# MaxRamgraber/Triangular-Transport-Toolbox

Measured on AMD Instinct MI355X. Metric: map-evals/sec (forward+inverse, N samples x D comps), higher is better.
Workload: dtype f64; 1 GPU; C5: d=40 banded separable map, order 3, N=1e6 (Gaussian-mixture target); N_per_gpu=1000000, D=40, columns=40, inverse=table, layout=column-major resident in HBM, coefficients=reference-optimised (tests/golden), world_size=1

## Files before the change

### triangular_transport_toolbox_amd/csrc/ttm_band.h

```cpp
#pragma once

#include <stdint.h>

#include "../../include/ttm.h"

namespace ttm_band {

int build_records(const ttm_program* p, double* U, void* stream);

int record_stride(int cls, int lag);

bool usable(const ttm_program* p, int k0, int k1);

int forward(const ttm_program* p, const double* U, int k0, int k1, const double* Xsoa, int64_t ldx, int64_t N, double* Zsoa,
            int64_t ldz, double* logdet, const double* sigma, double* sumsq, int cus, size_t lds_per_cu, int block, int resident, void* stream,
            const char** kernel_name);

int inverse(const ttm_program* p, const double* U, int k0, int k1, const double* Zsoa, int64_t ldz, double* Xsoa, int64_t ldx,
            int64_t N, const double* tab_x, int T, const double* y_affine, const double* tmin, const double* tmax, const int32_t* bkt,
            int nb, const double* img, int img_doubles, int cus, size_t lds_per_cu, int window, int block, int resident, void* stream,
            const char** kernel_name);

int newton(const ttm_program* p, const double* U, int k0, int k1, const double* Zsoa, int64_t ldz, double* Xsoa, int64_t ldx, int64_t N,
           int32_t* iters, int cus, size_t lds_per_cu, int block, void* stream, const char** kernel_name);

int bisect(const ttm_program* p, const double* U, int k0, int k1, const double* Zsoa, int64_t ldz, double* Xsoa, int64_t ldx, int64_t N,
           int32_t* iters, int cus, size_t lds_per_cu, int block, void* stream, const char** kernel_name);

bool bisect_plans(const ttm_program* p, const double* U, int k0, int k1, const double* Zsoa, int64_t ldz, double* Xsoa, int64_t ldx, int64_t N,
                  int32_t* iters, int cus, size_t lds_per_cu, int block);

int score(const ttm_program* p, const double* U, const double* Xsoa, int64_t ldx, int64_t N, double* Gsoa, int64_t ldg, const double* g_scale,
          const double* ld_affine, int cus, size_t lds_per_cu, int block, void* stream, const char** kernel_name);

int roundtrip(const ttm_program* p, const double* U, int k0, int k1, const double* Xsoa, int64_t ldx, int64_t N, double* Zsoa, int64_t ldz,
              double* Xr, int64_t ldr, double* logdet, const double* sigma, double* sumsq, const double* tab_x, int T, const double* y_affine,
// ... 9 lines not shown
```

### triangular_transport_toolbox_amd/csrc/ttm_band.hip

```cpp
#include <hip/hip_runtime.h>
#include <math.h>
#include <stdint.h>
#include <stdlib.h>
#include <type_traits>
#include <utility>

#include "ttm_band.h"
#include "ttm_band_etab.h"
#include "ttm_band_image.h"
#include "ttm_band_policy.h"

namespace ttm_band {

typedef const __attribute__((address_space(4))) double* cdbl_p;
typedef const __attribute__((address_space(4))) int* cint_p;
struct __attribute__((aligned(16))) D2 { double x, y; };

__device__ const double g_band_etab[2 * TTM_BAND_ET_N] = { TTM_BAND_ETAB_VALUES };
__device__ double g_band_taylor[6] = {1.0 / 5040.0, 1.0 / 720.0, 1.0 / 120.0, 1.0 / 24.0, 1.0 / 6.0, 0.5};

__host__ __device__ constexpr int cls_db(int cls) { return cls == 1 ? 3 : (cls == 2 ? 5 : (cls == 3 ? 7 : 10)); }
__host__ __device__ constexpr int cls_da(int cls) { return cls == 1 ? 1 : (cls == 2 ? 5 : (cls == 3 ? 7 : 10)); }
__host__ __device__ constexpr int cls_gs(int cls) { return cls == 1 ? 8 : (cls == 2 ? 16 : 24); }
__host__ __device__ constexpr int cls_gp(int cls) { return cls_db(cls) + 1 + cls_da(cls); }
__host__ __device__ constexpr int rec_stride(int cls, int lag) { return (TTM_P_HDR + lag * cls_gp(cls) + 7) / 8 * 8; }

#define BAND_ET_DOUBLES (2 * TTM_BAND_ET_N)
#define BAND_CT 1024
#define BAND_NS 4
#define BAND_PF 1
static_assert(BAND_POLICY_TILE_ROWS == BAND_NS * BAND_CT && BAND_POLICY_HALF_ROWS == 2 * BAND_CT && BAND_NS == 4,
              "ttm_band_policy.h counts the rows of pair slot 0 of these tiles");

__device__ __forceinline__ void band_dma16(const void* g, unsigned int lds_wave_base) {
    asm volatile("s_mov_b32 m0, %1\n\ts_nop 0\n\tglobal_load_lds_dwordx4 %0, off" ::"v"(g), "s"(lds_wave_base) : "m0");
}
__device__ __forceinline__ unsigned int band_lds_addr(const void* p) {
    return (unsigned int)(uintptr_t)(const __attribute__((address_space(3))) void*)p;
}

template <bool WAIT = true>
__device__ __forceinline__ void band_stage(double* lds_dst, const double* src, int n) {
    const int units = n >> 1;
    const unsigned int base = band_lds_addr(lds_dst);
    for (int u0 = 0; u0 < units; u0 += BAND_CT) {
        const int u = u0 + (int)threadIdx.x;
        if (u < units) band_dma16(src + 2 * (size_t)u, __builtin_amdgcn_readfirstlane(base + (unsigned int)(u0 + ((int)threadIdx.x & ~63)) * 16u));
    }
    if (WAIT) asm volatile("s_waitcnt vmcnt(0)" ::: "memory");
}
// ... 964 lines not shown
};

__device__ __forceinline__ void band_ring_fill(const double* img, int ncomp, double* tabs, int tab_slot, int n) {
    const int U = tab_slot >> 1;
    const int total = n * U;
    for (int u0 = 0; u0 < total; u0 += BAND_CT) {
        const int u = u0 + (int)threadIdx.x;
        if (u < total) {
            const int t = u / U, o = u - t * U;
            band_dma16(img + (size_t)(t % ncomp) * tab_slot + 2 * o,
                       __builtin_amdgcn_readfirstlane(band_lds_addr(tabs) + (unsigned int)(u0 + ((int)threadIdx.x & ~63)) * 16u));
        }
    }
}

template <int CLS, int LAG, bool RING = false, int G = 0, int POL = 0>
__device__ __forceinline__ void band_inverse_tile(const BandInvCtx& cx, bool full, int kb, int ke, const char* zcol, char* xcol, unsigned int tbase,
                                                  const unsigned int (&roff)[BAND_NS / 2], double (&pend)[BAND_NS][LAG],
                                                  const D2 (&zfirst)[BAND_NS / 2], bool have_first, BandRing* rg = nullptr) {
    constexpr int DB = cls_db(CLS), DA = cls_da(CLS), PS = rec_stride(CLS, LAG);
    constexpr int NS = BAND_NS, NP = NS / 2, HALF = 2 * BAND_CT;
    cdbl_p rec = cx.P + (int64_t)(kb + LAG) * PS;
    cdbl_p kt = cx.kt;
    const double* slot = RING ? cx.tabs + (size_t)rg->pos * cx.tab_slot : cx.tabs;
    const double ystep = cx.ystep;
    const int nb1 = cx.nb - 1;
    D2 za[NP], zb[NP];
    if (have_first) {
#pragma unroll
        for (int q = 0; q < NP; ++q) za[q] = zfirst[q];
    } else {
        band_slots<NP>([&](auto Q) { constexpr int q = decltype(Q)::value; za[q] = band_load2<band_z_nt<POL, q>>(zcol + roff[q]); });
    }
    auto interp = [&](double y_lo, double y_hi, double x_lo, double x_hi, double e_lo, double tgt, double& rr, double& ee) {
        const double dx = fmax(x_hi - x_lo, 1e-300);
        double rc = __builtin_amdgcn_rcp(dx);
        rc = fma(fma(-dx, rc, 1.0), rc, rc);
        const double delta = ((y_hi - y_lo) * rc) * (tgt - x_lo);
        rr = delta + y_lo;
        const double w = (delta * -0.25) * (y_lo + rr);
        double p = fma(kt[0], w, kt[1]);
        p = fma(p, w, kt[2]);
        p = fma(p, w, kt[3]);
        p = fma(p, w, kt[4]);
        p = fma(p, w, kt[5]);
        p = fma(p, w, 1.0);
        p = fma(p, w, 1.0);
        ee = e_lo * p;
    };
    auto step = [&](int j, const D2 (&zc)[NP], D2 (&zn)[NP]) {
        {
            const char* znext = j + 1 < ke ? zcol + cx.ldzb : zcol;
            band_slots<NP>([&](auto Q) { constexpr int q = decltype(Q)::value; zn[q] = band_load2<band_z_nt<POL, q>>(znext + roff[q]); });
        }
        double start = rec[1];
        double gc[LAG * (DB + 1 + DA)];
#pragma unroll
        for (int i = 0; i < LAG * (DB + 1 + DA); ++i) gc[i] = rec[TTM_P_HDR + i];
        asm volatile("" : "+s"(start));
#pragma unroll
        for (int i = 0; i < LAG * (DB + 1 + DA); ++i) asm volatile("" : "+s"(gc[i]));
        __builtin_amdgcn_sched_barrier(0);
        double wl, wh, scale, bias;
        { const D2 a = *(const D2*)slot; wl = a.x; wh = a.y; const D2 b = *(const D2*)(slot + 2); scale = b.x; bias = b.y; }
        const lds_p xsl = band_lds(slot + BAND_RT_HDR) - 8 * cx.w0;
        const lds_p bkl = band_lds(slot + BAND_RT_HDR + cx.Weven);
        const bool deg = __builtin_amdgcn_readfirstlane(((const int*)slot)[10]) != 0;
        const int per = __builtin_amdgcn_readfirstlane(((const int*)slot)[8]);
        double traw[NS], tg[NS], r[NS], E[NS];
        unsigned long long outl = deg ? ~0ull : 0ull;
#pragma unroll
        for (int e = 0; e < NS; ++e) {
            const double z = (e & 1) ? zc[e >> 1].y : zc[e >> 1].x;
            traw[e] = z - pend[e][0];
            tg[e] = fmin(fmax(traw[e], wl), wh);
            outl |= __builtin_amdgcn_ballot_w64(traw[e] != tg[e]);
        }
        if (RING && G > 0) {
            band_dma16(rg->src + (size_t)rg->tcomp * rg->stride, rg->tabs_lds + (unsigned int)rg->tpos * rg->stride + rg->dst);
            if (++rg->tpos == rg->R) rg->tpos = 0;
            if (++rg->tcomp == rg->ncomp) rg->tcomp = 0;
        }
        auto search = [&](auto nc) {
            constexpr int NC = decltype(nc)::value;
            int pos[NS];
#pragma unroll
            for (int e = 0; e < NS; ++e) {
                const int bi = min((int)fma(tg[e], scale, bias), nb1);
                pos[e] = (int)*(const __attribute__((address_space(3))) unsigned short*)(bkl + 2 * bi);
            }
            double qv[NS][NC];
#pragma unroll
            for (int e = 0; e < NS; ++e) {
                const lds_p q4 = xsl + 8 * pos[e];
                qv[e][0] = band_lds_f64(q4);
#pragma unroll
// ... 41 lines not shown
#pragma unroll
            for (int q = 0; q < NP; ++q) {
                band_store2<POL != 0>(xcol + (size_t)((tbase + (unsigned int)(q * HALF)) * 8u), r[2 * q], r[2 * q + 1]);
            }
        } else {
#pragma unroll
            for (int q = 0; q < NP; ++q) {
                const unsigned int n = tbase + (unsigned int)(q * HALF);
                const D2 o = {r[2 * q], r[2 * q + 1]};
                char* xp = xcol + (size_t)(n * 8u);
                if (n + 1 < cx.c1_32) { if (POL != 0) band_store2<true>(xp, o.x, o.y); else *(D2*)xp = o; }
                else if (n < cx.c1_32) *(double*)xp = o.x;
            }
        }
        rec += PS; slot += cx.tab_slot; zcol += cx.ldzb; xcol += cx.ldxb;
        if (RING) {
            if (++rg->pos == rg->R) { rg->pos = 0; slot = cx.tabs; }
            if (G > 0 && ++rg->gcnt == G) {
                rg->gcnt = 0;
                static_assert(G == 0 || G == 4, "the counted wait below is 3 G - 2");
                asm volatile("s_waitcnt vmcnt(10)" ::: "memory");
                __syncthreads();
            }
        }
    };
    int j = kb;
    for (; j + 1 < ke; j += 2) {
        step(j, za, zb);
        step(j + 1, zb, za);
    }
    if (j < ke) step(j, za, zb);
}

template <int CLS, int LAG, int KM>
__global__ __launch_bounds__(BAND_CT) void k_band_inverse(const double* __restrict__ U_, int64_t p_off, int k0, int k1, int kcol0,
                                                          const double* __restrict__ Z, int64_t ldz, double* X, int64_t ldx, int64_t N,
                                                          const double* __restrict__ tab_x, int T, double y0, double ystep, double ylast,
                                                          const double* __restrict__ tmin, const double* __restrict__ tmax,
                                                          const int* __restrict__ bkt, int nb, int tab_slot, int B, int64_t rows_per_wg,
                                                          int w0, int W) {
    constexpr int DB = cls_db(CLS), DA = cls_da(CLS), PS = rec_stride(CLS, LAG);
    constexpr int NS = BAND_NS, NP = NS / 2, CT = BAND_CT, ROWS = NS * CT, HALF = 2 * CT;
    extern __shared__ __align__(16) double g_lds[];
    const int tid = threadIdx.x;
    const int64_t c0 = (int64_t)blockIdx.x * rows_per_wg;
    if (c0 >= N) return;
// ... 129 lines not shown
                    for (int q = 0; q < NP; ++q) {
                        D2 xv = {0.0, 0.0};
                        if (cc >= 0) xv = *(const D2*)(col + roff[q]);
                        band_push<DB, DA, LAG>(rec + TTM_P_HDR, rec[1], xv.x, cc >= 0 ? band_expq_series(xv.x) : 1.0, pend[2 * q]);
                        band_push<DB, DA, LAG>(rec + TTM_P_HDR, rec[1], xv.y, cc >= 0 ? band_expq_series(xv.y) : 1.0, pend[2 * q + 1]);
                    }
                }
            }
            const char* zcol = (const char*)Z + (int64_t)(kb - k0) * ldzb;
            char* xcol = (char*)X + (int64_t)colb * ldxb;
            band_inverse_tile<CLS, LAG>(cx, full, kb, ke, zcol, xcol, tbase, roff, pend, zfirst, tile == 0);
        }
    }
}

template <int CLS, int LAG, int G, int POL = 0>
__global__ __launch_bounds__(BAND_CT) void k_band_inverse_ring(const double* __restrict__ U_, int64_t p_off, int k0, int k1, int kcol0,
                                                               const double* __restrict__ Z, int64_t ldz, double* X, int64_t ldx, int64_t N,
                                                               const double* __restrict__ tab_x, int T, double y0, double ystep, double ylast,
                                                               const double* __restrict__ tmin, const double* __restrict__ tmax,
                                                               const double* __restrict__ img, int nb, int tab_slot, int R,
                                                               int64_t rows_per_wg, int w0, int W) {
    constexpr int DB = cls_db(CLS), DA = cls_da(CLS), PS = rec_stride(CLS, LAG);
    constexpr int NS = BAND_NS, NP = NS / 2, CT = BAND_CT, ROWS = NS * CT, HALF = 2 * CT;
    extern __shared__ __align__(16) double g_lds[];
    const int tid = threadIdx.x;
    const int64_t c0 = (int64_t)blockIdx.x * rows_per_wg;
    if (c0 >= N) return;
    const int64_t c1 = c0 + rows_per_wg < N ? c0 + rows_per_wg : N;
    const int ntile = (int)((c1 - c0 + ROWS - 1) / ROWS);
    const int ncomp = k1 - k0;
// ... 10 lines not shown
    cx.T = T; cx.nb = nb; cx.tab_slot = tab_slot; cx.w0 = w0; cx.Weven = Weven; cx.k0 = k0;
    cx.y0 = y0; cx.ystep = ystep; cx.ylast = ylast; cx.ldzb = ldzb; cx.ldxb = ldxb; cx.c1_32 = (unsigned int)c1;
    BandRing rg;
    {
        const int U = tab_slot >> 1, nw = (U + 63) >> 6;
        const int piece = (tid >> 6) % nw;
        const int start = 64 * piece < U - 64 ? 64 * piece : U - 64;
        rg.src = (const char*)img + (size_t)(start + (tid & 63)) * 16;
        rg.dst = __builtin_amdgcn_readfirstlane((unsigned int)start * 16u);
        rg.tabs_lds = band_lds_addr(tabs);
        rg.stride = (unsigned int)tab_slot * 8u;
        rg.R = R; rg.ncomp = ncomp; rg.pos = 0; rg.gcnt = 0;
        rg.tpos = G > 0 ? R - G : 0;
        rg.tcomp = G > 0 ? (R - G) % ncomp : 0;
    }
    D2 zfirst[NP];
    band_slots<NP>([&](auto Q) {
        constexpr int q = decltype(Q)::value;
        unsigned int n = (unsigned int)c0 + 2u * (unsigned int)tid + (unsigned int)(q * HALF);
        n = n < last_pair ? n : last_pair;
        zfirst[q] = band_load2<band_z_nt<POL, q>>((const char*)Z + (size_t)(n * 8u));
    });
    band_ring_fill(img, ncomp, tabs, tab_slot, R);
    for (int i = tid; i < W; i += CT) {
        etab[2 * i] = band_expq_series(w0 + i == T - 1 ? ylast : (double)(w0 + i) * ystep + y0);
        etab[2 * i + 1] = w0 + i == T - 1 ? ylast : (double)(w0 + i) * ystep + y0;
    }
    asm volatile("s_waitcnt vmcnt(0)" ::: "memory");
    __syncthreads();
    for (int tile = 0; tile < ntile; ++tile) {
        const unsigned int tbase = (unsigned int)c0 + (unsigned int)tile * (unsigned int)ROWS + 2u * (unsigned int)tid;
        const bool full = c0 + (int64_t)(tile + 1) * ROWS <= c1;
        unsigned int roff[NP];
#pragma unroll
        for (int q = 0; q < NP; ++q) {
            unsigned int n = tbase + (unsigned int)(q * HALF);
            n = n < last_pair ? n : last_pair;
            roff[q] = n * 8u;
        }
        double pend[NS][LAG];
#pragma unroll
        for (int e = 0; e < NS; ++e)
#pragma unroll
            for (int l = 0; l < LAG; ++l) pend[e][l] = 0.0;
        for (int i = 0; i < LAG; ++i) {
            const int cc = kcol0 - LAG + i;
            cdbl_p rec = P + (int64_t)(k0 + i) * PS;
            const char* col = (const char*)X + (int64_t)(cc < 0 ? 0 : cc) * ldxb;
#pragma unroll
            for (int q = 0; q < NP; ++q) {
                D2 xv = {0.0, 0.0};
                if (cc >= 0) xv = *(const D2*)(col + roff[q]);
                band_push<DB, DA, LAG>(rec + TTM_P_HDR, rec[1], xv.x, cc >= 0 ? band_expq_series(xv.x) : 1.0, pend[2 * q]);
                band_push<DB, DA, LAG>(rec + TTM_P_HDR, rec[1], xv.y, cc >= 0 ? band_expq_series(xv.y) : 1.0, pend[2 * q + 1]);
            }
        }
        band_inverse_tile<CLS, LAG, true, G, POL>(cx, full, k0, k1, (const char*)Z, (char*)X + (int64_t)kcol0 * ldxb, tbase, roff, pend, zfirst, tile == 0, &rg);
    }
}

template <int CLS, int LAG, int LAGE, bool PLAIN>
__global__ __launch_bounds__(BAND_CT) void k_band_few_inverse(const double* __restrict__ U_, int64_t p_off, int k0, int k1, int kcol0,
                                                              const double* __restrict__ Z, int64_t ldz, double* X, int64_t ldx, int64_t N,
                                                              const double* __restrict__ tab_x, int T, double y0, double ystep, double ylast,
                                                              const double* __restrict__ tmin, const double* __restrict__ tmax,
                                                              const int* __restrict__ bkt, int nb, int tab_slot, int ntiles) {
    constexpr int DB = cls_db(CLS), DA = cls_da(CLS), GP = cls_gp(CLS), PS = rec_stride(CLS, LAG);
    constexpr int NS = BAND_FEW_NS, NP = NS / 2, CT = BAND_CT, ROWS = NS * CT, HALF = 2 * CT, FD = TTM_P_FEW_D, HDR = BAND_RT_HDR;
    extern __shared__ __align__(16) double g_lds[];
    const int tid = threadIdx.x;
    const int nc = k1 - k0;
// ... 1213 lines not shown
template <class F> static auto with_reach(int lag, int lage, F f) {
    if (lag == 5) return f(int_c<5>{}, int_c<5>{});
    if (lag == 3) return lage == 1 ? f(int_c<3>{}, int_c<1>{}) : lage == 2 ? f(int_c<3>{}, int_c<2>{}) : f(int_c<3>{}, int_c<3>{});
    return lage == 1 ? f(int_c<2>{}, int_c<1>{}) : f(int_c<2>{}, int_c<2>{});
}

static bool vec_ok(const void* ptr) { return (uintptr_t)ptr % 16 == 0; }
static bool col_ok(const void* ptr, int64_t ld, int64_t need) { return vec_ok(ptr) && ld % 2 == 0 && ld >= need; }
static int64_t even_rows(int64_t N) { return (N + 1) & ~(int64_t)1; }
static bool y_affine_ok(const double* y) {
    if (!y) return false;
    const double ymax = fabs(y[0]) > fabs(y[2]) ? fabs(y[0]) : fabs(y[2]);
    return y[1] > 0.0 && y[1] * ymax * 0.5 <= 0.1;
}

static int64_t chunk_rows(int64_t N, int cus) {
    const int64_t rows = (N + cus - 1) / cus;
    return (rows + 31) / 32 * 32;
}
struct ChunkGrid { int64_t rows, grid; };
static ChunkGrid chunk_grid(int64_t N, int cus) {
    const int64_t rows = chunk_rows(N, cus);
    return {rows, (N + rows - 1) / rows};
}

int record_stride(int cls, int lag) { return rec_stride(cls, lag); }

bool usable(const ttm_program* p, int k0, int k1) {
    return p && p->u_enabled && (p->u_p_lag == 2 || ((p->u_p_lag == 3 || p->u_p_lag == TTM_P_LAG_MAX) && p->D <= TTM_P_FEW_D)) && p->u_h_cls >= 1 &&
           (p->u_h_cls <= 3 || (p->u_h_cls == 4 && p->D <= TTM_P_FEW_D)) &&
           p->h_ucomp && k0 >= 0 && k1 <= p->D && k0 < k1 && p->u_p_stride == rec_stride(p->u_h_cls, p->u_p_lag);
}

static int uc(const ttm_program* p, int k, int word) { return p->h_ucomp[k * TTM_UC_LEN + word]; }
// ... 69 lines not shown
static size_t block_lds_span(const ttm_program* p, int k0, int k1, int Bc, bool splines_only) {
    size_t lds = 0;
    for (int kb = k0; kb < k1; kb += Bc) {
        int a = kb, b = (kb + Bc < k1 ? kb + Bc : k1) - 1;
        if (splines_only) {
            while (a <= b && uc(p, a, TTM_UC_NI) <= 0) ++a;
            while (b >= a && uc(p, b, TTM_UC_NI) <= 0) --b;
        }
        const size_t s = a > b ? 0 : (size_t)(uc(p, b, TTM_UC_TAB_OFF) + TTM_U_TSTRIDE * uc(p, b, TTM_UC_NI) - uc(p, a, TTM_UC_TAB_OFF)) * 8;
        lds = s > lds ? s : lds;
    }
    return lds;
}

int forward(const ttm_program* p, const double* U, int k0, int k1, const double* Xsoa, int64_t ldx, int64_t N, double* Zsoa, int64_t ldz,
            double* logdet, const double* sigma, double* sumsq, int cus, size_t lds_per_cu, int block, int resident, void* stream,
            const char** kernel_name) {
    if (!usable(p, k0, k1) || (!Zsoa && !logdet && !sumsq) || N >= ((int64_t)1 << 28)) return 1;
    if (!col_ok(Xsoa, ldx, even_rows(N)) || (Zsoa && !col_ok(Zsoa, ldz, 0)) || !vec_ok(U) || !vec_ok(logdet) || !vec_ok(sumsq)) return 1;
    const bool dens = logdet || sumsq;
    const size_t stat = dens ? (size_t)BAND_UNI * 8 : 0;
    if (dens && k1 - k0 > BAND_UNI) return 1;
    const size_t fixed = (size_t)BAND_ET_DOUBLES * 8 + stat;
    if (lds_per_cu <= fixed) return 1;
    const int Bc = plan_blocks(p, k0, k1, lds_per_cu - fixed, block);
    if (Bc <= 0) return 1;
    const size_t lds = block_lds_sum(p, k0, k1, Bc) + fixed - stat;
    const int cls = p->u_h_cls, lag = p->u_p_lag, kcol0 = uc(p, k0, TTM_UC_KC);
    if (logdet && !Zsoa && !sumsq && k1 - k0 <= BAND_UNI) {
        const size_t lbudget = lds_per_cu - (size_t)BAND_UNI * 8;
        const int LBc = plan_blocks(p, k0, k1, lbudget, block);
        const size_t llds = LBc > 0 ? block_lds_span(p, k0, k1, LBc, true) + 16 : 0;
// ... 23 lines not shown
                          ldx, N, Zsoa, ldz, logdet, sigma, sumsq, fs.ntiles, fs.tab0, fs.ntab);
        }
    }
    if (lag != 2 || cls > 3) return 1;
    const bool own = sweep_has_own(p, k0, k1);
    const ChunkGrid cg = chunk_grid(N, cus);
    if (dens) {
        auto dk = with_bool(Zsoa != nullptr, [&](auto WZ) {
            return with_bool(own, [&](auto OW) {
                return with_cls<3>(cls, [&](auto C) { return k_band_density<decltype(C)::value, 2, decltype(WZ)::value, decltype(OW)::value>; });
            });
        });
        return launch(dk, cg.grid, lds, stream, "k_band_density", kernel_name, U, p->u_p_off, k0, k1, kcol0, Xsoa, ldx, N, Zsoa, ldz, logdet, sigma,
                      sumsq, cg.rows, Bc);
    }
    const bool pol = (band_resident_policy(N, cg.rows, k1 - k0, resident) & BAND_POLICY_FORWARD) != 0;
    auto kern = with_bool(pol, [&](auto PO) {
        return with_bool(own, [&](auto OW) {
            return with_cls<3>(cls, [&](auto C) { return k_band_forward<decltype(C)::value, 2, decltype(OW)::value, decltype(PO)::value ? 1 : 0>; });
        });
    });
    return launch(kern, cg.grid, lds, stream, "k_band_forward", kernel_name, U, p->u_p_off, k0, k1, kcol0, Xsoa, ldx, N, Zsoa, ldz, cg.rows, Bc);
}

int roundtrip(const ttm_program* p, const double* U, int k0, int k1, const double* Xsoa, int64_t ldx, int64_t N, double* Zsoa, int64_t ldz,
              double* Xr, int64_t ldr, double* logdet, const double* sigma, double* sumsq, const double* tab_x, int T, const double* y_affine,
              const double* tmin, const double* tmax, const int32_t* bkt, int nb, int cus, size_t lds_per_cu, bool force, void* stream,
              const char** kernel_name) {
    const int nc = k1 - k0;
    if (!usable(p, k0, k1) || nc > TTM_P_FEW_D || !Xr || T < 64 || T + 4 > BAND_CT || nb + 1 != 1024 || N >= ((int64_t)1 << 28)) return 1;
    if (!vec_ok(bkt) || (sigma && !logdet) || !y_affine_ok(y_affine)) return 1;
    const int64_t need = even_rows(N);
    if (!col_ok(Xsoa, ldx, need) || (Zsoa && !col_ok(Zsoa, ldz, need)) || !col_ok(Xr, ldr, need) || !vec_ok(U) || !vec_ok(logdet) || !vec_ok(sumsq))
        return 1;
    const FewSweep fs = few_sweep(p, k0, k1, N, cus);
    const BandImageSlot slot = band_image_slot(T, nb);
    const size_t lds = slot.lds(nc) + fs.lds;
// ... 76 lines not shown
static BlockPlan block_plan(int T, int W, int nb, int ncomp, size_t lds_per_cu, int block) {
    const BandImageSlot slot = band_image_slot(W, nb);
    BlockPlan b = {W, (T - W) / 2, slot.tab_slot, 0, 0, 0};
    if (slot.lds(1) > lds_per_cu) return b;
    b.Bc = (int)((lds_per_cu - slot.lds(0)) / ((size_t)slot.tab_slot * 8));
    if (b.Bc > ncomp) b.Bc = ncomp;
    if (b.Bc > BAND_RT_KMAX) b.Bc = BAND_RT_KMAX;
    if (block > 0 && block < b.Bc) b.Bc = block;
    b.nblk = (ncomp + b.Bc - 1) / b.Bc;
    b.lds = slot.lds(b.Bc);
    return b;
}

int inverse(const ttm_program* p, const double* U, int k0, int k1, const double* Zsoa, int64_t ldz, double* Xsoa, int64_t ldx, int64_t N,
            const double* tab_x, int T, const double* y_affine, const double* tmin, const double* tmax, const int32_t* bkt, int nb, const double* img,
            int img_doubles, int cus, size_t lds_per_cu, int window, int block, int resident, void* stream, const char** kernel_name) {
    if (!usable(p, k0, k1) || T < 64 || T > 4096 || nb + 1 != 1024 || N >= ((int64_t)1 << 28)) return 1;
    if (!vec_ok(bkt) || !y_affine_ok(y_affine)) return 1;
    if (!col_ok(Zsoa, ldz, even_rows(N)) || !col_ok(Xsoa, ldx, even_rows(N))) return 1;
    const int ncomp = k1 - k0, cls = p->u_h_cls, lag = p->u_p_lag, kcol0 = uc(p, k0, TTM_UC_KC);
    if (ncomp <= TTM_P_FEW_D && T + 4 <= BAND_CT && window <= 0) {
        const BandImageSlot slot = band_image_slot(T, nb);
        const FewSweep fs = few_sweep(p, k0, k1, N, cus);
        if (slot.lds(ncomp) <= lds_per_cu && fs.lage <= lag) {
            auto fk = with_reach(lag, fs.lage, [&](auto L, auto E) {
                return with_bool(fs.plain, [&](auto PL) {
                    return with_cls<4>(cls, [&](auto C) {
                        return k_band_few_inverse<decltype(C)::value, decltype(L)::value, decltype(E)::value, decltype(PL)::value>;
                    });
                });
            });
            return launch(fk, fs.grid, slot.lds(ncomp), stream, "k_band_few_inverse", kernel_name, U, p->u_p_off, k0, k1, kcol0, Zsoa, ldz, Xsoa, ldx,
                          N, tab_x, T, y_affine[0], y_affine[1], y_affine[2], tmin, tmax, bkt, nb, slot.tab_slot, fs.ntiles);
        }
    }
    if (lag != 2 || cls > 3) return 1;
    const ChunkGrid cg = chunk_grid(N, cus);
    BandRingPlan pl;
    if (img && vec_ok(img) && band_ring_plan(T, nb, ncomp, lds_per_cu, window, block, BAND_WFRAC, &pl) &&
        pl.tab_slot == img_doubles) {
        const bool pol = (band_resident_policy(N, cg.rows, ncomp, resident) & BAND_POLICY_INVERSE) != 0;
        auto rk = with_bool(pol, [&](auto PO) {
            return with_bool(pl.G == 4, [&](auto G4) {
                return with_cls<3>(cls, [&](auto C) {
                    return k_band_inverse_ring<decltype(C)::value, 2, decltype(G4)::value ? 4 : 0, decltype(PO)::value ? 1 : 0>;
                });
            });
        });
        return launch(rk, cg.grid, pl.lds, stream, "k_band_inverse_ring", kernel_name, U, p->u_p_off, k0, k1, kcol0, Zsoa, ldz, Xsoa, ldx, N, tab_x, T,
                      y_affine[0], y_affine[1], y_affine[2], tmin, tmax, img, nb, pl.tab_slot, pl.R, cg.rows, pl.w0, pl.W);
    }
    BlockPlan b = block_plan(T, T, nb, ncomp, lds_per_cu, block);
    if (window != 0 && (window > 0 || (b.Bc > 0 && b.nblk > 1))) {
        int W = window > 0 ? (window < 16 ? 16 : window) : (int)(BAND_WFRAC * T);
        if (W >= T) W = T - 1;
        const BlockPlan w = block_plan(T, W, nb, ncomp, lds_per_cu, block);
        if (w.Bc > 0 && (window > 0 || w.nblk < b.nblk)) b = w;
    }
    if (b.Bc <= 0) return 1;
    auto kern = with_cls<3>(cls, [&](auto C) { return k_band_inverse<decltype(C)::value, 2, BAND_RT_KMAX>; });
    return launch(kern, cg.grid, b.lds, stream, "k_band_inverse", kernel_name, U, p->u_p_off, k0, k1, kcol0, Zsoa, ldz, Xsoa, ldx, N, tab_x, T,
                  y_affine[0], y_affine[1], y_affine[2], tmin, tmax, bkt, nb, b.tab_slot, b.Bc, cg.rows, b.w0, b.W);
}

int score(const ttm_program* p, const double* U, const double* Xsoa, int64_t ldx, int64_t N, double* Gsoa, int64_t ldg, const double* g_scale,
// ... 30 lines not shown
```

### triangular_transport_toolbox_amd/csrc/ttm_band_image.h

```cpp
#pragma once

#include <math.h>
#include <stddef.h>
#include <stdint.h>

#define BAND_RT_HDR 6
#define BAND_RING_KMAX 24

struct BandImageSlot {
    int Weven, tab_slot;
    size_t lds(int slots) const { return ((size_t)2 * Weven + (size_t)slots * tab_slot) * 8; }
};
static inline BandImageSlot band_image_slot(int W, int nb) {
    const int Weven = (W + 4 + 1) & ~1;
    return {Weven, BAND_RT_HDR + Weven + (((nb + 1 + 3) / 4 + 1) & ~1)};
}

struct BandRingPlan {
    int W, w0, Weven, tab_slot;
    int R, G;
    size_t lds;
};

static inline bool band_ring_plan(int T, int nb, int ncomp, size_t lds_per_cu, int window, int block, double wfrac, BandRingPlan* pl) {
// ... 19 lines not shown
    pl->W = W; pl->w0 = w0;
    const BandImageSlot slot = band_image_slot(W, nb);
    pl->Weven = slot.Weven; pl->tab_slot = slot.tab_slot;
    if (pl->tab_slot % 2) return false;
    if (ncomp <= B) { pl->R = ncomp; pl->G = 0; }
    else {
        const int G = 4;
        const int R = B / G * G;
        if (R < 3 * G) return false;
        pl->R = R; pl->G = G;
    }
    pl->lds = slot.lds(pl->R);
    return true;
}

#if defined(__HIPCC__)
__device__ __forceinline__ void band_bucket_params(double lo, double hi, int nb, double& scale, double& bias) {
    scale = (double)nb / (hi - lo);
    if (!(scale > 0.0 && scale < 1.0e300)) scale = 0.0;
    bias = -lo * scale;
}

__device__ inline void band_image_write(const double* xs, const int* bks, int* red, int T, int nb, double lo, double hi, int w0, int W,
                                        int Weven, int tab_slot, double* __restrict__ img) {
    const int tid = threadIdx.x, nt = blockDim.x;
    if (tid == 0) *red = 0;
    __syncthreads();
    int per = 0;
    for (int b = tid; b < nb; b += nt) {
        const int b0 = bks[b] & 0xffff, b1 = bks[b + 1] & 0xffff;
// ... 31 lines not shown
```

### triangular_transport_toolbox_amd/csrc/ttm_band_policy.h

```cpp
#pragma once

#include <stdint.h>

constexpr int64_t TTM_LLC_BYTES = (int64_t)256 << 20;

constexpr int BAND_POLICY_TILE_ROWS = 4096;
constexpr int BAND_POLICY_HALF_ROWS = 2048;

constexpr int BAND_POLICY_FORWARD = 1;
constexpr int BAND_POLICY_INVERSE = 2;

static inline int64_t band_policy_resident_rows(int64_t N, int64_t chunk_rows) {
    if (N <= 0 || chunk_rows <= 0) return 0;
    auto of_chunk = [](int64_t n) {
        const int64_t tail = n % BAND_POLICY_TILE_ROWS;
        return n / BAND_POLICY_TILE_ROWS * BAND_POLICY_HALF_ROWS + (tail < BAND_POLICY_HALF_ROWS ? tail : BAND_POLICY_HALF_ROWS);
    };
    const int64_t whole = N / chunk_rows;
    return whole * of_chunk(chunk_rows) + of_chunk(N - whole * chunk_rows);
}

static inline int band_resident_policy(int64_t N, int64_t chunk_rows, int ncomp, int option) {
    if (option >= 0) return option & (BAND_POLICY_FORWARD | BAND_POLICY_INVERSE);
    const int64_t col = 8 * (int64_t)ncomp;
    if (col * N <= TTM_LLC_BYTES) return 0;
    if (band_policy_resident_rows(N, chunk_rows) * col > TTM_LLC_BYTES) return 0;
    return BAND_POLICY_FORWARD | BAND_POLICY_INVERSE;
}
```

### triangular_transport_toolbox_amd/csrc/ttm_kernels.hip

```cpp

#include <hip/hip_runtime.h>
#include <mutex>

#include <stdio.h>
#include <stdlib.h>
#include <string.h>

#include <type_traits>

#include "ttm_eval.h"
#include "ttm_dev.h"
#include "ttm_dense.h"
#include "ttm_sample_logq.h"
#include "ttm_rng.h"
#include "ttm_uform.h"
#include "ttm_score.h"
#include "ttm_band.h"
#include "ttm_band_image.h"
#include "ttm_int.h"
#include "ttm_options.h"

using namespace ttm;


// ... 3192 lines not shown
        const int chunk = (k1 - k0 + nchunk - 1) / nchunk;
        if (ibd && ttm_int::forward(p, dev_prog(p), k0, k1, coef, fold, Xsoa, ldx, N, Zsoa, ldz, logdet, sigma, sumsq, tiles, chunk, ibd,
                                    lds_bytes(nsl, ibd, 0, 1), tuning().int_xprog != 0, stream, &name) == TTM_OK)
            return check_launch(name);
    }
    if (sep && u_on(p) && all_fast(p, k0, k1) && N < ((int64_t)1 << 29)) {
        int tab_cap = 0;
        for (int k = k0; k < k1; ++k) {
            const int c = TTM_U_TSTRIDE * p->h_ucomp[k * TTM_UC_LEN + TTM_UC_NI];
            tab_cap = c > tab_cap ? c : tab_cap;
        }
        const int ways = plan_ways_of(p);
        if (band_forward_gate(p, k0, k1, N)) {
            const char* name = nullptr;
            if (ttm_band::forward(p, fold + fold_base_size(p), k0, k1, Xsoa, ldx, N, Zsoa, ldz, logdet, sigma, sumsq, band_cus(),
                                  device_info().lds_per_cu, tuning().rt_block, tuning().band_resident, stream, &name) == 0)
                return check_launch(name);
        }
        {
            int nimax = 0, nchmax = 0;
            for (int k = k0; k < k1; ++k) {
                const int ni = p->h_ucomp[k * TTM_UC_LEN + TTM_UC_NI];
                nimax = ni > nimax ? ni : nimax;
            }
            nchmax = (nimax * TTM_U_TSTRIDE * 8 + 1023) >> 10;
            const int tab_slot = TTM_U_TSTRIDE * nimax;
            int xlead = 3, tlead = 2;
            const Tuning& tn = tuning();
            int hNS = 4;
            if (tn.hl_ns > 0) hNS = tn.hl_ns == 4 ? 4 : 2;
            const bool hot = hot_sweepable(p) && !tn.u_no_hot;
// ... 245 lines not shown
                      int64_t ldz, double* Xsoa, int64_t ldx, int64_t N, const double* tab_x, const double* tab_y, int64_t ldy,
                      int32_t T, const double* h_y_affine, const double* tmin, const double* tmax, const int32_t* bkt, int32_t nb,
                      int32_t truncate, const double* img, int64_t img_doubles, void* stream) {
    int rc = validate(p, k0, k1);
    if (rc) return rc;
    if (!coef || !fold || !Zsoa || !Xsoa || !tab_x || !tab_y || !tmin || !tmax || !bkt || N < 1 || ldx < N || ldz < N || T < 2 ||
        T < 8 || T > 65536 || nb < 4 || nb > 65536 || (ldy != 0 && ldy < T) || (h_y_affine && ldy != 0))
        return set_err(TTM_E_ARG, "ttm_inverse_table: bad arguments%s");
    if (p->monotonicity != TTM_MONO_SEPARABLE) return set_err(TTM_E_UNSUPPORTED, "table inverse needs separable monotonicity%s");
    const Tuning& tn = tuning();
    const bool affine = h_y_affine && ldy == 0;
    if (affine && truncate && band_inverse_gate(p, k0, k1, N, T, nb)) {
        const char* name = nullptr;
        if (ttm_band::inverse(p, fold + fold_base_size(p), k0, k1, Zsoa, ldz, Xsoa, ldx, N, tab_x, (int)T, h_y_affine, tmin, tmax, bkt, (int)nb,
                              tn.band_ring != 0 ? img : nullptr, (int)img_doubles, band_cus(), device_info().lds_per_cu, tn.rt_window, tn.rt_block,
                              tn.band_resident, stream, &name) == 0)
            return check_launch(name);
    }
    if (affine && rt_inverse_gate(p, k0, k1, N, T, nb) && hot_sweepable(p) && (k1 - k0 >= 4 || tn.u_loader == 1)) {
        const DeviceInfo& di = device_info();
        const int ways = plan_ways_of(p);
        const int ncomp = k1 - k0;
        int NS = tn.rt_ns == 4 ? 4 : 2;
        int W = T, w0 = 0;
        int Weven = (W + 4 + 1) & ~1;
        int tab_slot = TTM_RT_HDR + Weven + (((nb + 1 + 3) / 4 + 1) & ~1);
        const double ymax = fabs(h_y_affine[0]) > fabs(h_y_affine[2]) ? fabs(h_y_affine[0]) : fabs(h_y_affine[2]);
        const bool etab = truncate && h_y_affine[1] > 0.0 && h_y_affine[1] * ymax * 0.5 <= 0.1;
        const bool aligned = ((uintptr_t)Zsoa % 16 == 0) && (ldz % 2 == 0) && ldz >= ((N + 1) & ~(int64_t)1) &&
                             ((uintptr_t)Xsoa % 16 == 0) && (ldx % 2 == 0) && ldx >= ((N + 1) & ~(int64_t)1);
        bool band = p->u_h_ng == 2 && tn.rt_band != 0;
// ... 686 lines not shown
```

### triangular_transport_toolbox_amd/csrc/ttm_options.h

```cpp
#pragma once

#include <string.h>

#define TTM_OPTIONS(X)                                                                                                   \
    X(no_plan, 0)         \
    X(no_uform, 0)        \
    X(u_no_hot, 0)        \
    X(u_loader, -1)       \
    X(forward_ns, -1)     \
    X(inverse_ns, -1)     \
    X(u_ns, -1)           \
    X(hl_ns, -1)          \
    X(rt_off, 0)          \
    X(rt_ns, -1)          \
    X(rt_block, -1)       \
    X(rt_band, -1)        \
    X(rt_window, -1)      \
    X(gram_mfma, -1)      \
    X(band_fwd, -1)       \
    X(band_inv, -1)       \
    X(band_cus, -1)       \
    X(band_ring, -1)      \
    X(band_newton, -1)    \
    X(band_bisect, -1)    \
    X(band_score, -1)     \
    X(band_resident, -1)  \
    X(int_dense, -1)      \
    X(int_xprog, -1)      \
    X(fold_fused, -1)     \
    X(table_fused, -1)    \
    X(setup_fused, -1)    \
    X(select_coop, -1)    \
    X(colstats_one, -1)   \
    X(sep_sentinel, -1)   \
    X(sep_server, -1)     \
    X(wscan_reread, -1)   \
    X(roundtrip_fused, -1)

struct Tuning {
#define X(name, dflt) int name = dflt;
    TTM_OPTIONS(X)
// ... 10 lines not shown
```

Baseline: 162.6 billion map-evals/s.

## Add full-tile row cut and LDS-staged Z prefetch for band ring inverse

Adds a launch cut that gives each workgroup exactly one full tile of rows when the tile count nearly matches the CU count. This lets the forward and ring-inverse kernels take the full-tile code path instead of partial chunks. Also adds an opt-in variant of the ring inverse that double-buffers Z columns into LDS with async global-to-LDS loads and counted waits, trading ring slots for LDS space. The Z-DMA path and the ring-slot override are off by default; the full-tile cut is on by default, at the cost of slightly fewer workgroups than CUs.

```diff
diff --git a/triangular_transport_toolbox_amd/csrc/ttm_band.h b/triangular_transport_toolbox_amd/csrc/ttm_band.h
--- a/triangular_transport_toolbox_amd/csrc/ttm_band.h
+++ b/triangular_transport_toolbox_amd/csrc/ttm_band.h
@@ -13,13 +13,13 @@
 bool usable(const ttm_program* p, int k0, int k1);
 
 int forward(const ttm_program* p, const double* U, int k0, int k1, const double* Xsoa, int64_t ldx, int64_t N, double* Zsoa,
-            int64_t ldz, double* logdet, const double* sigma, double* sumsq, int cus, size_t lds_per_cu, int block, int resident, void* stream,
-            const char** kernel_name);
+            int64_t ldz, double* logdet, const double* sigma, double* sumsq, int cus, size_t lds_per_cu, int block, int resident, int full_tiles,
+            void* stream, const char** kernel_name);
 
 int inverse(const ttm_program* p, const double* U, int k0, int k1, const double* Zsoa, int64_t ldz, double* Xsoa, int64_t ldx,
             int64_t N, const double* tab_x, int T, const double* y_affine, const double* tmin, const double* tmax, const int32_t* bkt,
-            int nb, const double* img, int img_doubles, int cus, size_t lds_per_cu, int window, int block, int resident, void* stream,
-            const char** kernel_name);
+            int nb, const double* img, int img_doubles, int cus, size_t lds_per_cu, int window, int block, int resident, int full_tiles, int zdma,
+            int ring_slots, void* stream, const char** kernel_name);
 
 int newton(const ttm_program* p, const double* U, int k0, int k1, const double* Zsoa, int64_t ldz, double* Xsoa, int64_t ldx, int64_t N,
            int32_t* iters, int cus, size_t lds_per_cu, int block, void* stream, const char** kernel_name);
diff --git a/triangular_transport_toolbox_amd/csrc/ttm_band.hip b/triangular_transport_toolbox_amd/csrc/ttm_band.hip
--- a/triangular_transport_toolbox_amd/csrc/ttm_band.hip
+++ b/triangular_transport_toolbox_amd/csrc/ttm_band.hip
@@ -34,6 +34,9 @@
 
 __device__ __forceinline__ void band_dma16(const void* g, unsigned int lds_wave_base) {
     asm volatile("s_mov_b32 m0, %1\n\ts_nop 0\n\tglobal_load_lds_dwordx4 %0, off" ::"v"(g), "s"(lds_wave_base) : "m0");
+}
+__device__ __forceinline__ void band_dma16_nt(const void* g, unsigned int lds_wave_base) {
+    asm volatile("s_mov_b32 m0, %1\n\ts_nop 0\n\tglobal_load_lds_dwordx4 %0, off nt" ::"v"(g), "s"(lds_wave_base) : "m0");
 }
 __device__ __forceinline__ unsigned int band_lds_addr(const void* p) {
     return (unsigned int)(uintptr_t)(const __attribute__((address_space(3))) void*)p;
@@ -1028,10 +1031,17 @@
     }
 }
 
-template <int CLS, int LAG, bool RING = false, int G = 0, int POL = 0>
+#define BAND_ZD_BUF (BAND_NS * BAND_CT * 8)
+static_assert(2 * BAND_ZD_BUF == BAND_ZDMA_LDS_BYTES, "ttm_band_policy.h counts the LDS of these two buffers");
+template <int POL, int Q>
+__device__ __forceinline__ void band_zd_request(const char* g, unsigned int lds_wave_base) {
+    if (band_z_nt<POL, Q>) band_dma16_nt(g, lds_wave_base); else band_dma16(g, lds_wave_base);
+}
+template <int CLS, int LAG, bool RING = false, int G = 0, int POL = 0, int ZD = 0>
 __device__ __forceinline__ void band_inverse_tile(const BandInvCtx& cx, bool full, int kb, int ke, const char* zcol, char* xcol, unsigned int tbase,
                                                   const unsigned int (&roff)[BAND_NS / 2], double (&pend)[BAND_NS][LAG],
-                                                  const D2 (&zfirst)[BAND_NS / 2], bool have_first, BandRing* rg = nullptr) {
+                                                  const D2 (&zfirst)[BAND_NS / 2], bool have_first, BandRing* rg = nullptr, unsigned int zq = 0) {
+    static_assert(ZD == 0 || (RING && POL == 1), "ZD = 1: the ring kernel under the resident policy");
     constexpr int DB = cls_db(CLS), DA = cls_da(CLS), PS = rec_stride(CLS, LAG);
     constexpr int NS = BAND_NS, NP = NS / 2, HALF = 2 * BAND_CT;
     cdbl_p rec = cx.P + (int64_t)(kb + LAG) * PS;
@@ -1040,7 +1050,16 @@
     const double ystep = cx.ystep;
     const int nb1 = cx.nb - 1;
     D2 za[NP], zb[NP];
-    if (have_first) {
+    auto zrd = [&]() {
+        unsigned int a;
+        asm volatile("v_mbcnt_lo_u32_b32 %0, -1, 0\n\tv_mbcnt_hi_u32_b32 %0, -1, %0\n\tv_lshl_add_u32 %0, %0, 4, %1" : "=&v"(a) : "s"(zq));
+        return (lds_p)(uintptr_t)a;
+    };
+    if (ZD) {
+#pragma unroll
+        for (int q = 0; q < NP; ++q) za[q] = band_lds_pair(zrd() + q * 1024);
+        asm volatile("s_waitcnt lgkmcnt(0)" ::: "memory");
+    } else if (have_first) {
 #pragma unroll
         for (int q = 0; q < NP; ++q) za[q] = zfirst[q];
     } else {
@@ -1062,8 +1081,14 @@
         p = fma(p, w, 1.0);
         ee = e_lo * p;
     };
-    auto step = [&](int j, const D2 (&zc)[NP], D2 (&zn)[NP]) {
-        {
+    auto step = [&](int j, const D2 (&zc)[NP], D2 (&zn)[NP], int par) {
+        if (ZD) {
+            const char* zreq = zcol + (j + 2 < ke ? 2 * cx.ldzb : j + 1 < ke ? cx.ldzb : 0);
+            band_slots<NP>([&](auto Q) {
+                constexpr int q = decltype(Q)::value;
+                band_zd_request<POL, q>(zreq + roff[q], zq + (unsigned int)(par * BAND_ZD_BUF + q * 1024));
+            });
+        } else {
             const char* znext = j + 1 < ke ? zcol + cx.ldzb : zcol;
             band_slots<NP>([&](auto Q) { constexpr int q = decltype(Q)::value; zn[q] = band_load2<band_z_nt<POL, q>>(znext + roff[q]); });
         }
@@ -1094,6 +1119,15 @@
             band_dma16(rg->src + (size_t)rg->tcomp * rg->stride, rg->tabs_lds + (unsigned int)rg->tpos * rg->stride + rg->dst);
             if (++rg->tpos == rg->R) rg->tpos = 0;
             if (++rg->tcomp == rg->ncomp) rg->tcomp = 0;
+        }
+        if (ZD) {
+            constexpr int PIECE = G > 0 ? 1 : 0, BEHIND = (PIECE + 2) + (2 + PIECE);
+            static_assert(BEHIND == (G > 0 ? 6 : 4), "the literal of the counted wait below");
+            if (G > 0) asm volatile("s_waitcnt vmcnt(6)" ::: "memory");
+            else asm volatile("s_waitcnt vmcnt(4)" ::: "memory");
+            const lds_p zr = zrd();
+#pragma unroll
+            for (int q = 0; q < NP; ++q) zn[q] = band_lds_pair(zr + ((par ^ 1) * BAND_ZD_BUF + q * 1024));
         }
         auto search = [&](auto nc) {
             constexpr int NC = decltype(nc)::value;
@@ -1165,22 +1199,24 @@
             }
         }
         rec += PS; slot += cx.tab_slot; zcol += cx.ldzb; xcol += cx.ldxb;
+        if (ZD) asm volatile("s_waitcnt lgkmcnt(0)" ::: "memory");
         if (RING) {
             if (++rg->pos == rg->R) { rg->pos = 0; slot = cx.tabs; }
             if (G > 0 && ++rg->gcnt == G) {
                 rg->gcnt = 0;
-                static_assert(G == 0 || G == 4, "the counted wait below is 3 G - 2");
-                asm volatile("s_waitcnt vmcnt(10)" ::: "memory");
+                static_assert(G == 0 || (3 * G - 2 == 10 && (2 + 1 + 2) * G + 2 == 22), "the literals of the counted waits below: 3 G - 2 and 5 G + 2");
+                if (ZD) asm volatile("s_waitcnt vmcnt(22)" ::: "memory");
+                else asm volatile("s_waitcnt vmcnt(10)" ::: "memory");
                 __syncthreads();
             }
         }
     };
     int j = kb;
     for (; j + 1 < ke; j += 2) {
-        step(j, za, zb);
-        step(j + 1, zb, za);
-    }
-    if (j < ke) step(j, za, zb);
+        step(j, za, zb, 0);
+        step(j + 1, zb, za, 1);
+    }
+    if (j < ke) step(j, za, zb, 0);
 }
 
 template <int CLS, int LAG, int KM>
@@ -1340,7 +1376,7 @@
     }
 }
 
-template <int CLS, int LAG, int G, int POL = 0>
+template <int CLS, int LAG, int G, int POL = 0, int ZD = 0>
 __global__ __launch_bounds__(BAND_CT) void k_band_inverse_ring(const double* __restrict__ U_, int64_t p_off, int k0, int k1, int kcol0,
                                                                const double* __restrict__ Z, int64_t ldz, double* X, int64_t ldx, int64_t N,
                                                                const double* __restrict__ tab_x, int T, double y0, double ystep, double ylast,
@@ -1381,7 +1417,23 @@
         rg.tpos = G > 0 ? R - G : 0;
         rg.tcomp = G > 0 ? (R - G) % ncomp : 0;
     }
+    const unsigned int zq = ZD ? __builtin_amdgcn_readfirstlane(band_lds_addr(etab + 2 * Weven) + (unsigned int)(tid >> 6) * 2048u) : 0u;
+    auto zd_request2 = [&](int tile) {
+        band_slots<NP>([&](auto Q) {
+            constexpr int q = decltype(Q)::value;
+            const unsigned int n = (unsigned int)c0 + (unsigned int)tile * (unsigned int)ROWS + 2u * (unsigned int)tid + (unsigned int)(q * HALF);
+            const char* g = (const char*)Z + (size_t)(n * 8u);
+            band_zd_request<POL, q>(g, zq + (unsigned int)(q * 1024));
+            band_zd_request<POL, q>(k0 + 1 < k1 ? g + ldzb : g, zq + (unsigned int)(BAND_ZD_BUF + q * 1024));
+        });
+    };
+    const bool zd0 = ZD != 0 && c0 + ROWS <= c1;
     D2 zfirst[NP];
+    if (zd0) {
+        zd_request2(0);
+#pragma unroll
+        for (int q = 0; q < NP; ++q) zfirst[q] = D2{0.0, 0.0};
+    } else
     band_slots<NP>([&](auto Q) {
         constexpr int q = decltype(Q)::value;
         unsigned int n = (unsigned int)c0 + 2u * (unsigned int)tid + (unsigned int)(q * HALF);
@@ -1405,6 +1457,10 @@
             n = n < last_pair ? n : last_pair;
             roff[q] = n * 8u;
         }
+        if (ZD && full && tile > 0) {
+            asm volatile("s_waitcnt vmcnt(0)" ::: "memory");
+            zd_request2(tile);
+        }
         double pend[NS][LAG];
 #pragma unroll
         for (int e = 0; e < NS; ++e)
@@ -1422,6 +1478,12 @@
                 band_push<DB, DA, LAG>(rec + TTM_P_HDR, rec[1], xv.y, cc >= 0 ? band_expq_series(xv.y) : 1.0, pend[2 * q + 1]);
             }
         }
+        if (ZD && full) {
+            if constexpr (ZD != 0) {
+                if (tile > 0) asm volatile("s_waitcnt vmcnt(0)" ::: "memory");
+                band_inverse_tile<CLS, LAG, true, G, POL, 1>(cx, true, k0, k1, (const char*)Z, (char*)X + (int64_t)kcol0 * ldxb, tbase, roff, pend, zfirst, false, &rg, zq);
+            }
+        } else
         band_inverse_tile<CLS, LAG, true, G, POL>(cx, full, k0, k1, (const char*)Z, (char*)X + (int64_t)kcol0 * ldxb, tbase, roff, pend, zfirst, tile == 0, &rg);
     }
 }
@@ -2665,10 +2727,7 @@
     return y[1] > 0.0 && y[1] * ymax * 0.5 <= 0.1;
 }
 
-static int64_t chunk_rows(int64_t N, int cus) {
-    const int64_t rows = (N + cus - 1) / cus;
-    return (rows + 31) / 32 * 32;
-}
+static int64_t chunk_rows(int64_t N, int cus) { return band_policy_chunk_rows(N, cus); }
 struct ChunkGrid { int64_t rows, grid; };
 static ChunkGrid chunk_grid(int64_t N, int cus) {
     const int64_t rows = chunk_rows(N, cus);
@@ -2768,8 +2827,8 @@
 }
 
 int forward(const ttm_program* p, const double* U, int k0, int k1, const double* Xsoa, int64_t ldx, int64_t N, double* Zsoa, int64_t ldz,
-            double* logdet, const double* sigma, double* sumsq, int cus, size_t lds_per_cu, int block, int resident, void* stream,
-            const char** kernel_name) {
+            double* logdet, const double* sigma, double* sumsq, int cus, size_t lds_per_cu, int block, int resident, int full_tiles,
+            void* stream, const char** kernel_name) {
     if (!usable(p, k0, k1) || (!Zsoa && !logdet && !sumsq) || N >= ((int64_t)1 << 28)) return 1;
     if (!col_ok(Xsoa, ldx, even_rows(N)) || (Zsoa && !col_ok(Zsoa, ldz, 0)) || !vec_ok(U) || !vec_ok(logdet) || !vec_ok(sumsq)) return 1;
     const bool dens = logdet || sumsq;
@@ -2823,13 +2882,14 @@
         return launch(dk, cg.grid, lds, stream, "k_band_density", kernel_name, U, p->u_p_off, k0, k1, kcol0, Xsoa, ldx, N, Zsoa, ldz, logdet, sigma,
                       sumsq, cg.rows, Bc);
     }
-    const bool pol = (band_resident_policy(N, cg.rows, k1 - k0, resident) & BAND_POLICY_FORWARD) != 0;
+    const BandCut lc = band_policy_cut(N, cus, full_tiles);
+    const bool pol = (band_resident_policy(N, lc.rows, k1 - k0, resident) & BAND_POLICY_FORWARD) != 0;
     auto kern = with_bool(pol, [&](auto PO) {
         return with_bool(own, [&](auto OW) {
             return with_cls<3>(cls, [&](auto C) { return k_band_forward<decltype(C)::value, 2, decltype(OW)::value, decltype(PO)::value ? 1 : 0>; });
         });
     });
-    return launch(kern, cg.grid, lds, stream, "k_band_forward", kernel_name, U, p->u_p_off, k0, k1, kcol0, Xsoa, ldx, N, Zsoa, ldz, cg.rows, Bc);
+    return launch(kern, lc.grid, lds, stream, "k_band_forward", kernel_name, U, p->u_p_off, k0, k1, kcol0, Xsoa, ldx, N, Zsoa, ldz, lc.rows, Bc);
 }
 
 int roundtrip(const ttm_program* p, const double* U, int k0, int k1, const double* Xsoa, int64_t ldx, int64_t N, double* Zsoa, int64_t ldz,
@@ -2936,7 +2996,8 @@
 
 int inverse(const ttm_program* p, const double* U, int k0, int k1, const double* Zsoa, int64_t ldz, double* Xsoa, int64_t ldx, int64_t N,
             const double* tab_x, int T, const double* y_affine, const double* tmin, const double* tmax, const int32_t* bkt, int nb, const double* img,
-            int img_doubles, int cus, size_t lds_per_cu, int window, int block, int resident, void* stream, const char** kernel_name) {
+            int img_doubles, int cus, size_t lds_per_cu, int window, int block, int resident, int full_tiles, int zdma, int ring_slots,
+            void* stream, const char** kernel_name) {
     if (!usable(p, k0, k1) || T < 64 || T > 4096 || nb + 1 != 1024 || N >= ((int64_t)1 << 28)) return 1;
     if (!vec_ok(bkt) || !y_affine_ok(y_affine)) return 1;
     if (!col_ok(Zsoa, ldz, even_rows(N)) || !col_ok(Xsoa, ldx, even_rows(N))) return 1;
@@ -2961,16 +3022,18 @@
     BandRingPlan pl;
     if (img && vec_ok(img) && band_ring_plan(T, nb, ncomp, lds_per_cu, window, block, BAND_WFRAC, &pl) &&
         pl.tab_slot == img_doubles) {
-        const bool pol = (band_resident_policy(N, cg.rows, ncomp, resident) & BAND_POLICY_INVERSE) != 0;
-        auto rk = with_bool(pol, [&](auto PO) {
-            return with_bool(pl.G == 4, [&](auto G4) {
-                return with_cls<3>(cls, [&](auto C) {
-                    return k_band_inverse_ring<decltype(C)::value, 2, decltype(G4)::value ? 4 : 0, decltype(PO)::value ? 1 : 0>;
-                });
+        const BandRingLaunch rl = band_ring_launch(pl, N, cus, ncomp, lds_per_cu, full_tiles, resident, zdma, ring_slots);
+        const BandCut lc = rl.cut;
+        const bool pol = rl.pol, zd = rl.zd;
+        pl = rl.ring;
+        auto rk = with_bool(pl.G == 4, [&](auto G4) {
+            return with_cls<3>(cls, [&](auto C) {
+                constexpr int CL = decltype(C)::value, GG = decltype(G4)::value ? 4 : 0;
+                return zd ? k_band_inverse_ring<CL, 2, GG, 1, 1> : pol ? k_band_inverse_ring<CL, 2, GG, 1> : k_band_inverse_ring<CL, 2, GG>;
             });
         });
-        return launch(rk, cg.grid, pl.lds, stream, "k_band_inverse_ring", kernel_name, U, p->u_p_off, k0, k1, kcol0, Zsoa, ldz, Xsoa, ldx, N, tab_x, T,
-                      y_affine[0], y_affine[1], y_affine[2], tmin, tmax, img, nb, pl.tab_slot, pl.R, cg.rows, pl.w0, pl.W);
+        return launch(rk, lc.grid, pl.lds, stream, "k_band_inverse_ring", kernel_name, U, p->u_p_off, k0, k1, kcol0, Zsoa, ldz, Xsoa, ldx, N, tab_x, T,
+                      y_affine[0], y_affine[1], y_affine[2], tmin, tmax, img, nb, pl.tab_slot, pl.R, lc.rows, pl.w0, pl.W);
     }
     BlockPlan b = block_plan(T, T, nb, ncomp, lds_per_cu, block);
     if (window != 0 && (window > 0 || (b.Bc > 0 && b.nblk > 1))) {
diff --git a/triangular_transport_toolbox_amd/csrc/ttm_band_image.h b/triangular_transport_toolbox_amd/csrc/ttm_band_image.h
--- a/triangular_transport_toolbox_amd/csrc/ttm_band_image.h
+++ b/triangular_transport_toolbox_amd/csrc/ttm_band_image.h
@@ -3,6 +3,8 @@
 #include <math.h>
 #include <stddef.h>
 #include <stdint.h>
+
+#include "ttm_band_policy.h"
 
 #define BAND_RT_HDR 6
 #define BAND_RING_KMAX 24
@@ -57,6 +59,40 @@
     return true;
 }
 
+static inline bool band_ring_plan_with(const BandRingPlan& pl, size_t lds_per_cu, size_t extra, int max_slots, BandRingPlan* out) {
+    const BandImageSlot slot = {pl.Weven, pl.tab_slot};
+    if (slot.lds(0) + extra > lds_per_cu) return false;
+    const int B = (int)((lds_per_cu - extra - slot.lds(0)) / ((size_t)slot.tab_slot * 8));
+    *out = pl;
+    if (pl.G == 0) { if (B < pl.R) return false; }
+    else {
+        int R = (B < pl.R ? B : pl.R) / pl.G * pl.G;
+        if (R < 3 * pl.G) return false;
+        if (max_slots > 0 && max_slots < R) R = (max_slots < 3 * pl.G ? 3 * pl.G : max_slots) / pl.G * pl.G;
+        out->R = R;
+    }
+    out->lds = slot.lds(out->R) + extra;
+    return true;
+}
+
+struct BandRingLaunch {
+    BandCut cut;
+    bool pol, zd;
+    BandRingPlan ring;
+};
+static inline BandRingLaunch band_ring_launch(const BandRingPlan& pl, int64_t N, int cus, int ncomp, size_t lds_per_cu, int full_tiles,
+                                              int resident, int zdma, int ring_slots) {
+    BandRingLaunch l;
+    l.cut = band_policy_cut(N, cus, full_tiles);
+    l.pol = (band_resident_policy(N, l.cut.rows, ncomp, resident) & BAND_POLICY_INVERSE) != 0;
+    const int slots = ring_slots > 0 ? ring_slots : 0;
+    BandRingPlan with;
+    l.zd = band_zdma_policy(N, l.cut, l.pol, band_ring_plan_with(pl, lds_per_cu, (size_t)BAND_ZDMA_LDS_BYTES, slots, &with), zdma);
+    l.ring = pl;
+    if (l.zd || (slots > 0 && band_ring_plan_with(pl, lds_per_cu, 0, slots, &with))) l.ring = with;
+    return l;
+}
+
 #if defined(__HIPCC__)
 __device__ __forceinline__ void band_bucket_params(double lo, double hi, int nb, double& scale, double& bias) {
     scale = (double)nb / (hi - lo);
diff --git a/triangular_transport_toolbox_amd/csrc/ttm_band_policy.h b/triangular_transport_toolbox_amd/csrc/ttm_band_policy.h
--- a/triangular_transport_toolbox_amd/csrc/ttm_band_policy.h
+++ b/triangular_transport_toolbox_amd/csrc/ttm_band_policy.h
@@ -20,6 +20,27 @@
     return whole * of_chunk(chunk_rows) + of_chunk(N - whole * chunk_rows);
 }
 
+struct BandCut { int64_t rows, grid; bool full_tiles; };
+static inline int64_t band_policy_chunk_rows(int64_t N, int cus) {
+    const int64_t rows = (N + cus - 1) / cus;
+    return (rows + 31) / 32 * 32;
+}
+static inline BandCut band_policy_cut(int64_t N, int cus, int option) {
+    if (cus < 1) cus = 1;
+    const int64_t tiles = (N + BAND_POLICY_TILE_ROWS - 1) / BAND_POLICY_TILE_ROWS;
+    const bool fits = N > 0 && tiles <= cus;
+    if (option != 0 && fits && (option > 0 || tiles >= cus - cus / 16)) return {BAND_POLICY_TILE_ROWS, tiles, true};
+    const int64_t rows = band_policy_chunk_rows(N, cus);
+    return {rows, rows > 0 ? (N + rows - 1) / rows : 0, false};
+}
+
+constexpr int64_t BAND_ZDMA_LDS_BYTES = 2 * (int64_t)BAND_POLICY_TILE_ROWS * 8;
+static inline bool band_zdma_policy(int64_t N, BandCut cut, bool pol_inverse, bool ring_ok, int option) {
+    if (option <= 0 || !pol_inverse || !ring_ok) return false;
+    return N >= BAND_POLICY_TILE_ROWS && cut.rows >= BAND_POLICY_TILE_ROWS;
+}
+
+
 static inline int band_resident_policy(int64_t N, int64_t chunk_rows, int ncomp, int option) {
     if (option >= 0) return option & (BAND_POLICY_FORWARD | BAND_POLICY_INVERSE);
     const int64_t col = 8 * (int64_t)ncomp;
diff --git a/triangular_transport_toolbox_amd/csrc/ttm_kernels.hip b/triangular_transport_toolbox_amd/csrc/ttm_kernels.hip
--- a/triangular_transport_toolbox_amd/csrc/ttm_kernels.hip
+++ b/triangular_transport_toolbox_amd/csrc/ttm_kernels.hip
@@ -3230,7 +3230,7 @@
         if (band_forward_gate(p, k0, k1, N)) {
             const char* name = nullptr;
             if (ttm_band::forward(p, fold + fold_base_size(p), k0, k1, Xsoa, ldx, N, Zsoa, ldz, logdet, sigma, sumsq, band_cus(),
-                                  device_info().lds_per_cu, tuning().rt_block, tuning().band_resident, stream, &name) == 0)
+                                  device_info().lds_per_cu, tuning().rt_block, tuning().band_resident, tuning().band_full_tiles, stream, &name) == 0)
                 return check_launch(name);
         }
         {
@@ -3506,7 +3506,7 @@
         const char* name = nullptr;
         if (ttm_band::inverse(p, fold + fold_base_size(p), k0, k1, Zsoa, ldz, Xsoa, ldx, N, tab_x, (int)T, h_y_affine, tmin, tmax, bkt, (int)nb,
                               tn.band_ring != 0 ? img : nullptr, (int)img_doubles, band_cus(), device_info().lds_per_cu, tn.rt_window, tn.rt_block,
-                              tn.band_resident, stream, &name) == 0)
+                              tn.band_resident, tn.band_full_tiles, tn.band_zdma, tn.band_ring_slots, stream, &name) == 0)
             return check_launch(name);
     }
     if (affine && rt_inverse_gate(p, k0, k1, N, T, nb) && hot_sweepable(p) && (k1 - k0 >= 4 || tn.u_loader == 1)) {
diff --git a/triangular_transport_toolbox_amd/csrc/ttm_options.h b/triangular_transport_toolbox_amd/csrc/ttm_options.h
--- a/triangular_transport_toolbox_amd/csrc/ttm_options.h
+++ b/triangular_transport_toolbox_amd/csrc/ttm_options.h
@@ -25,6 +25,9 @@
     X(band_bisect, -1)    \
     X(band_score, -1)     \
     X(band_resident, -1)  \
+    X(band_full_tiles, -1)  \
+    X(band_zdma, -1)      \
+    X(band_ring_slots, -1)  \
     X(int_dense, -1)      \
     X(int_xprog, -1)      \
     X(fold_fused, -1)     \
```

New measurement: 168.3 billion map-evals/s, median of 6. +3.5%, better.
